# lollcat/fab-torch

Measured on AMD Instinct MI355X. Metric: AIS samples/sec (+ESS), ManyWell-32, 8 intermediate dists, higher is better.
Workload: dtype f32; 1 GPU; headline: ManyWell-32 AIS, RealNVP 10x(16-320-320-32)+InvAffine (seeded default init, last coupling Linears N(0, 0.01^2)), HMC L=5 n_outer=1, M=8 linear beta, alpha=2 (target p^2/q), step-size tuning on; chains_per_gpu=1024, global_chains=1024, parallelism=single GPU

## Files before the change

fab_torch_amd/csrc/flow_r4.h:

```cpp
#pragma once
#include "flow_device.h"
#include "target_device.h"

namespace fab {

constexpr int R4 = 4;
constexpr int R4_DS = MAX_DIM + 4;

struct R4Dims {
    int Kd, Ko, KD;
    int G;
    int o_AW, o_AWT, o_W1, o_W2, o_W3, o_W3T, o_W2T, o_W1T, layer_stride;
};

FAB_HD R4Dims make_r4_dims(const FlowDims& f) {
    R4Dims r;
    r.Kd = pad16(f.d); r.Ko = pad16(2 * f.DOp); r.KD = pad16(f.D);
    r.G = f.Wp / 64;
    int o = 0;
    r.o_AW = o; o += r.KD * 64;
    r.o_AWT = o; o += r.KD * 64;
    r.o_W1 = o; o += r.Kd * f.Wp;
    r.o_W2 = o; o += f.Wp * f.Wp;
    r.o_W3 = o; o += f.Wp * 2 * f.DOp;
    r.o_W3T = o; o += r.Ko * f.Wp;
    r.o_W2T = o; o += f.Wp * f.Wp;
    r.o_W1T = o; o += f.Wp * pad16(f.d);
    r.layer_stride = o;
    return r;
}

struct R4Lds {
    int WS, PN;
    int o_X0, o_X1, o_HA, o_HB, o_PRM, o_DP, o_PART, o_ES, o_V2, o_MASK, total;
    int o_PZ, o_BIAS;
    int o_PF;
};

FAB_HD R4Lds make_r4_lds(const FlowDims& f, bool fused = false) {
    R4Lds l;
    l.WS = fused ? f.Wp + 16 : f.Wp + 4;
    l.PN = f.Wp;
    int o = 0;
    l.o_X0 = o; o += R4 * R4_DS;
    l.o_X1 = o; o += R4 * R4_DS;
    l.o_HA = o; o += R4 * l.WS;
    l.o_HB = o; o += R4 * l.WS;
    l.o_PRM = o; o += R4 * R4_DS;
    l.o_DP = o; o += R4 * R4_DS;
    l.o_PART = o; o += NWAVE * R4 * l.PN;
    l.o_ES = o; o += f.K * R4 * f.DOp;
    l.o_V2 = o; o += f.K * R4 * f.DOp;
    l.o_MASK = o; o += f.K * 2 * NTHREADS;
    l.o_PZ = l.o_BIAS = l.o_PF = 0;
    if (fused) {
        o = (o + 3) & ~3;
        l.o_PZ = o; o += 2 * NWAVE * R4 * 32;
        l.o_BIAS = o; o += (f.K + 1) * r4f_bias_stride(f.Wp);
        o = (o + 3) & ~3;
        l.o_PF = o; o += NWAVE * 64;
    }
    l.total = (o + 3) & ~3;
    return l;
}

__device__ __forceinline__ f32x4 mfma44(float a, float b, f32x4 c) {
    return __builtin_amdgcn_mfma_f32_4x4x1f32(a, b, c, 0, 0, 0);
}

struct Tid4 {
    int tid, wave, lane, arow;
    __device__ __forceinline__ Tid4() {
        tid = threadIdx.x;
        wave = __builtin_amdgcn_readfirstlane(tid >> 6);
        lane = tid & 63;
        arow = lane & 3;
    }
};

template <int NQ, int G>
struct R4Pre {
    float4 b[NQ][G];
};

template <int NQ, int G>
__device__ __forceinline__ void r4_preload(R4Pre<NQ, G>& p, const float4* __restrict__ Bm, int qbase, int nq_valid,
                                           const Tid4& t) {
    const float4* bw = Bm + ((size_t)qbase * G) * 64 + t.lane;
#pragma unroll
    for (int q = 0; q < NQ; ++q)
#pragma unroll
        for (int g = 0; g < G; ++g)
            if (q < nq_valid) p.b[q][g] = bw[(size_t)(q * G + g) * 64];
}

__device__ __forceinline__ void r4_barrier() { asm volatile("s_waitcnt lgkmcnt(0)\n\ts_barrier" ::: "memory"); }

template <int Q0, int Q1, int NQ, int G>
__device__ __forceinline__ void r4_preload_part(R4Pre<NQ, G>& p, const float4* __restrict__ Bm, int qbase, const Tid4& t) {
    const float4* bw = Bm + ((size_t)qbase * G) * 64 + t.lane;
#pragma unroll
    for (int q = Q0; q < Q1 && q < NQ; ++q)
#pragma unroll
        for (int g = 0; g < G; ++g) p.b[q][g] = bw[(size_t)(q * G + g) * 64];
}

struct R4NoNext {
    __device__ __forceinline__ void operator()() const {}
};

template <int G, class BT>
__device__ __forceinline__ void r4_quad(const float4& a, const BT (&b)[G], f32x4 (&acc)[G]) {
#pragma unroll
    for (int g = 0; g < G; ++g) acc[g] = mfma44(a.x, b[g].x, acc[g]);
#pragma unroll
    for (int g = 0; g < G; ++g) acc[g] = mfma44(a.y, b[g].y, acc[g]);
#pragma unroll
    for (int g = 0; g < G; ++g) acc[g] = mfma44(a.z, b[g].z, acc[g]);
#pragma unroll
    for (int g = 0; g < G; ++g) acc[g] = mfma44(a.w, b[g].w, acc[g]);
}

template <int NTWM>
struct R4Ring {
    static constexpr int NQ = 4 * NTWM, RD = NQ < 6 ? NQ : 6;
};

template <int NTWM, int G, class Next>
__device__ __forceinline__ void r4_mma_wide(const float* __restrict__ act, int lda, const float4* __restrict__ Bm,
                                            const R4Pre<R4Ring<NTWM>::RD, G>& pre, const Tid4& t, f32x4 (&acc)[G], Next next) {
    constexpr int NQ = R4Ring<NTWM>::NQ, RD = R4Ring<NTWM>::RD;
    const float* arow = act + t.arow * lda + 16 * NTWM * t.wave;
    const float4* bw = Bm + ((size_t)(4 * NTWM * t.wave) * G) * 64 + t.lane;
    float4 b[RD][G];
#pragma unroll
    for (int q = 0; q < RD; ++q)
#pragma unroll
        for (int g = 0; g < G; ++g) b[q][g] = pre.b[q][g];
    next();
    __builtin_amdgcn_sched_barrier(0);
#pragma unroll
    for (int q = 0; q < NQ; ++q) {
        const float4 a = *reinterpret_cast<const float4*>(arow + 4 * q);
        r4_quad<G>(a, b[q % RD], acc);
        if (q + RD < NQ) {
#pragma unroll
            for (int g = 0; g < G; ++g) b[q % RD][g] = bw[(size_t)((q + RD) * G + g) * 64];
        }
        __builtin_amdgcn_sched_barrier(0);
    }
}

template <int G>
__device__ __forceinline__ void r4_store_part(const f32x4 (&acc)[G], float* __restrict__ part, int PN, const Tid4& t) {
    float* pw = part + (size_t)t.wave * R4 * PN + t.lane;
#pragma unroll
    for (int g = 0; g < G; ++g)
#pragma unroll
        for (int r = 0; r < 4; ++r) pw[r * PN + 64 * g] = acc[g][r];
}

template <int G>
__device__ __forceinline__ void r4_bias_load(float (&bv)[G], const float* __restrict__ bias, const Tid4& t) {
    constexpr int N = 64 * G;
#pragma unroll
    for (int i = 0; i < G; ++i) bv[i] = bias ? bias[(256 * i + t.tid) % N] : 0.f;
}

typedef float f32x2 __attribute__((ext_vector_type(2)));
template <int O0, int O1>
__device__ __forceinline__ f32x2 lds_read2st64(unsigned addr) {
    f32x2 v;
    asm volatile("ds_read2st64_b32 %0, %1 offset0:%2 offset1:%3" : "=v"(v) : "v"(addr), "n"(O0), "n"(O1) : "memory");
    return v;
}
template <int G>
__device__ __forceinline__ void r4_read_partials(const float* part, int PN, int tid, float (&v)[G]) {
    (void)PN;
    const unsigned addr = (unsigned)(size_t)(part + tid);
    f32x2 r[2 * G];
    static_for<0, G>([&](auto ic) {
        constexpr int i = decltype(ic)::value;
        r[2 * i] = lds_read2st64<4 * i, 4 * i + 8 * G>(addr);
        r[2 * i + 1] = lds_read2st64<4 * i + 4 * G, 4 * i + 12 * G>(addr);
    });
    asm volatile("s_waitcnt lgkmcnt(0)" ::: "memory");
#pragma unroll
    for (int k = 0; k < 2 * G; ++k) asm volatile("" : "+v"(r[k]));
#pragma unroll
    for (int i = 0; i < G; ++i) {
        const f32x2 h = r[2 * i] + r[2 * i + 1];
        v[i] = h.x + h.y;
    }
}

struct R4NoPost {
    __device__ __forceinline__ float operator()(int, int, float v) const { return v; }
};

template <int G, int EP, class Post = R4NoPost>
__device__ __forceinline__ void r4_epilogue(const float* __restrict__ part, int PN, const float (&bv)[G],
                                            float* __restrict__ out, int ldo, unsigned* mask, const Tid4& t,
                                            Post post = Post()) {
    constexpr int N = 64 * G;
    unsigned m = EP == 2 ? mask[t.tid] : 0u;
    float v[G];
    if constexpr (G >= 2) {
        r4_read_partials<G>(part, PN, t.tid, v);
#pragma unroll
        for (int i = 0; i < G; ++i) v[i] += bv[i];
    } else {
#pragma unroll
        for (int i = 0; i < G; ++i) {
            const int o = 256 * i + t.tid, row = o / N, col = o - row * N;
            const float* p = part + row * PN + col;
            v[i] = ((p[0] + p[R4 * PN]) + (p[2 * R4 * PN] + p[3 * R4 * PN])) + bv[i];
        }
    }
#pragma unroll
    for (int i = 0; i < G; ++i) {
        const int o = 256 * i + t.tid, row = o / N, col = o - row * N;
        float w = v[i];
        if (EP == 1) { const bool pos = w > 0.f; m |= (pos ? 1u : 0u) << i; w = pos ? w : 0.f; }
        if (EP == 2) w = ((m >> i) & 1u) ? w : 0.f;
        out[row * ldo + col] = post(row, col, w);
    }
    if (EP == 1) mask[t.tid] = m;
}

template <int G>
__device__ __forceinline__ void r4_store_part_rf(const f32x4 (&acc)[G], float* __restrict__ part, const Tid4& t) {
    f32x4* pw = reinterpret_cast<f32x4*>(part + (size_t)t.wave * R4 * 64 * G) + t.lane;
#pragma unroll
    for (int g = 0; g < G; ++g) pw[64 * g] = acc[g];
}
template <int G>
__device__ __forceinline__ void r4_bias_rf(float (&bv)[G], const float* __restrict__ b, const Tid4& t) {
#pragma unroll
    for (int i = 0; i < G; ++i) bv[i] = b[(256 * i + t.tid) >> 2];
}
template <int G, int EP>
__device__ __forceinline__ void r4_epilogue_rf(const float* __restrict__ part, const float (&bv)[G], float* __restrict__ out, int ldo,
                                               unsigned* mask, const Tid4& t) {
    unsigned m = EP == 2 ? mask[t.tid] : 0u;
    float v[G];
    r4_read_partials<G>(part, 64 * G, t.tid, v);
    const int row = t.tid & 3, col0 = t.tid >> 2;
#pragma unroll
    for (int i = 0; i < G; ++i) {
        float w = v[i] + bv[i];
        if (EP == 1) { const bool pos = w > 0.f; m |= (pos ? 1u : 0u) << i; w = pos ? w : 0.f; }
        if (EP == 2) w = ((m >> i) & 1u) ? w : 0.f;
        out[row * ldo + col0 + 64 * i] = w;
    }
    if (EP == 1) mask[t.tid] = m;
}

template <int NTWM, int G, int EP, class Next = R4NoNext>
__device__ __forceinline__ void r4_dense_wide(const float* act, int lda, const float4* Bm,
                                              const R4Pre<R4Ring<NTWM>::RD, G>& pre,
                                              const float (&bv)[G], float* out, int ldo, unsigned* mask, float* part, int PN,
                                              const Tid4& t, Next next = Next()) {
    f32x4 acc[G];
#pragma unroll
    for (int g = 0; g < G; ++g) acc[g] = (f32x4){0.f, 0.f, 0.f, 0.f};
    r4_mma_wide<NTWM, G>(act, lda, Bm, pre, t, acc, next);
    r4_store_part<G>(acc, part, PN, t);
    r4_barrier();
    r4_epilogue<G, EP>(part, PN, bv, out, ldo, mask, t);
    r4_barrier();
}

template <int NTWM, int NT>
struct R4PreT {
    float4 b[NTWM][NT];
};

template <int NTWM, int NT>
__device__ __forceinline__ void r4_preload_n16(R4PreT<NTWM, NT>& p, const float4* __restrict__ Bm, const Tid4& t) {
    const float4* bw = Bm + ((size_t)(NTWM * t.wave) * NT) * 64 + t.lane;
#pragma unroll
    for (int Q = 0; Q < NTWM; ++Q)
#pragma unroll
        for (int ct = 0; ct < NT; ++ct) p.b[Q][ct] = bw[(size_t)(Q * NT + ct) * 64];
}

template <int NTWM, int NT, bool ACC = false, class Next = R4NoNext>
__device__ __forceinline__ void r4_dense_n16(const float* act, int lda, const R4PreT<NTWM, NT>& pre, float* out, int ldo,
                                             float* part, int PN, const Tid4& t, Next next = Next()) {
    constexpr int NSUB = 4 / NT, CW = 16 * NT, NTILE = NTWM * NT;
    static_assert(NT == 1 || NT == 2 || NT == 4, "16, 32 or 64 output columns");
    const int sblk = t.lane / CW, col = t.lane % CW;
    const float* arow = act + t.arow * lda + 16 * NTWM * t.wave + 4 * sblk;
    f32x4 acc0 = (f32x4){0.f, 0.f, 0.f, 0.f}, acc1 = acc0;
#pragma unroll
    for (int T = 0; T < NTILE; ++T) {
        const float4 a = *reinterpret_cast<const float4*>(arow + 4 * NSUB * T);
        const float4 w = pre.b[T / NT][T % NT];
        acc0 = mfma44(a.x, w.x, acc0);
        acc1 = mfma44(a.y, w.y, acc1);
        acc0 = mfma44(a.z, w.z, acc0);
        acc1 = mfma44(a.w, w.w, acc1);
    }
    next();
    acc0 += acc1;
    (void)PN;
    float* pw = part + ((size_t)(t.wave * NSUB + sblk) * R4) * CW + col;
#pragma unroll
    for (int r = 0; r < 4; ++r) pw[r * CW] = acc0[r];
    r4_barrier();
    if (t.tid < R4 * CW) {
        const int row = t.tid / CW, c = t.tid - row * CW;
        const float* p = part + row * CW + c;
        float v[4 * NSUB];
#pragma unroll
        for (int i = 0; i < 4 * NSUB; ++i) v[i] = p[(size_t)i * R4 * CW];
#pragma unroll
        for (int n = 4 * NSUB; n > 1; n >>= 1)
#pragma unroll
            for (int i = 0; i < n / 2; ++i) v[i] = v[2 * i] + v[2 * i + 1];
        if (ACC) out[row * ldo + c] += v[0];
        else out[row * ldo + c] = v[0];
    }
    r4_barrier();
}

template <int NQ, int G, int EP, class Next = R4NoNext, class Post = R4NoPost>
__device__ __forceinline__ void r4_dense_short(const float* act, int lda, int kmax, int nqw, const R4Pre<NQ, G>& pre,
                                               const float (&bv)[G], float* out, int ldo, unsigned* mask, float* part, int PN,
                                               const Tid4& t, Next next = Next(), Post post = Post()) {
    f32x4 acc[G];
#pragma unroll
    for (int g = 0; g < G; ++g) acc[g] = (f32x4){0.f, 0.f, 0.f, 0.f};
    const int q0 = nqw * t.wave;
#pragma unroll
    for (int q = 0; q < NQ; ++q) {
        if (q < nqw) {
            const int k0 = 4 * (q0 + q);
            float4 a = *reinterpret_cast<const float4*>(act + t.arow * lda + k0);
            if (k0 + 0 >= kmax) a.x = 0.f;
            if (k0 + 1 >= kmax) a.y = 0.f;
            if (k0 + 2 >= kmax) a.z = 0.f;
            if (k0 + 3 >= kmax) a.w = 0.f;
            r4_quad<G>(a, pre.b[q], acc);
        }
    }
    next();
    r4_store_part<G>(acc, part, PN, t);
    r4_barrier();
    r4_epilogue<G, EP>(part, PN, bv, out, ldo, mask, t, post);
    r4_barrier();
}

template <int NTWM, int NQS, int NQA, int NT3, int NT1>
__device__ float flow_log_prob_r4(const FlowDims& f, const R4Dims& rd, const R4Lds& l, const float* __restrict__ packed,
                                  float* lds, const Tid4& t, int* grad_off) {
    constexpr int G = NTWM;
    const float* r4base = packed + f.o_r4;
    int cur = l.o_X0, nxt = l.o_X1;
    float* HA = lds + l.o_HA;
    float* HB = lds + l.o_HB;
    float* PRM = lds + l.o_PRM;
    float* DP = lds + l.o_DP;
    float* PART = lds + l.o_PART;
    const bool ew = t.tid < 64;
    const int row = t.tid >> 4, c = t.tid & 15;
    const int nqD = rd.KD / 16, nqd = rd.Kd / 16, nqo = rd.Ko / 16;
    const int qW = 4 * NTWM * t.wave;
    R4Pre<NQA, 1> preA;
    R4PreT<NTWM, NT3> preN3;
    R4PreT<NTWM, NT1> preN1;
    R4Pre<NQS, G> preS;
    constexpr int RD = R4Ring<NTWM>::RD;
    R4Pre<RD, G> preW;
    float bvA[1], bv1[G], bv2[G], bv0[G];
#pragma unroll
    for (int g = 0; g < G; ++g) bv0[g] = 0.f;
    float logq = 0.f;
    {
        const float* Lp = packed + (size_t)(f.K - 1) * f.layer_stride;
        const float* Rp = r4base + (size_t)(f.K - 1) * rd.layer_stride;
        r4_preload<NQA, 1>(preA, reinterpret_cast<const float4*>(Rp + rd.o_AW), nqD * t.wave, nqD, t);
        r4_preload<NQS, G>(preS, reinterpret_cast<const float4*>(Rp + rd.o_W1), nqd * t.wave, nqd, t);
        r4_bias_load<1>(bvA, Lp + f.o_ac, t);
        r4_bias_load<G>(bv1, Lp + f.o_b1, t);
        r4_preload_part<0, 3>(preW, reinterpret_cast<const float4*>(Rp + rd.o_W2), qW, t);
    }
    for (int layer = f.K - 1; layer >= 0; --layer) {
        const float* Lp = packed + (size_t)layer * f.layer_stride;
        const float* Rp = r4base + (size_t)layer * rd.layer_stride;
        unsigned* mk = reinterpret_cast<unsigned*>(lds + l.o_MASK) + (size_t)layer * 2 * NTHREADS;
        const bool tl = layer == f.K - 2;
        if (tl) FAB_TL(f, 0);
        r4_dense_short<NQA, 1, 0>(lds + cur, R4_DS, f.D, nqD, preA, bvA, lds + nxt, R4_DS, nullptr, PART, l.PN, t, [&] {
            r4_preload_part<3, 5>(preW, reinterpret_cast<const float4*>(Rp + rd.o_W2), qW, t);
        });
        logq += Lp[f.o_logS];
        float* Z = lds + nxt;
        if (tl) FAB_TL(f, 1);
        r4_dense_short<NQS, G, 1>(Z, R4_DS, f.d, nqd, preS, bv1, HA, l.WS, mk, PART, l.PN, t, [&] {
            r4_preload_part<5, RD>(preW, reinterpret_cast<const float4*>(Rp + rd.o_W2), qW, t);
        });
        if (tl) FAB_TL(f, 2);
        float b3s[2] = {0.f, 0.f}, b3c[2] = {0.f, 0.f};
        r4_bias_load<G>(bv2, Lp + f.o_b2, t);
        r4_dense_wide<NTWM, G, 1>(HA, l.WS, reinterpret_cast<const float4*>(Rp + rd.o_W2), preW, bv2, HB, l.WS,
                                  mk + NTHREADS, PART, l.PN, t, [&] {
            r4_preload_n16<NTWM, NT3>(preN3, reinterpret_cast<const float4*>(Rp + rd.o_W3), t);
#pragma unroll
            for (int it = 0; it < 2; ++it) {
                const int j = c + 16 * it;
                if (ew && j < f.DO) { b3s[it] = Lp[f.o_b3 + j]; b3c[it] = Lp[f.o_b3 + f.DOp + j]; }
            }
            if (layer > 0) {
                const float* Ln = Lp - f.layer_stride;
                const float* Rn = Rp - rd.layer_stride;
                r4_preload<NQA, 1>(preA, reinterpret_cast<const float4*>(Rn + rd.o_AW), nqD * t.wave, nqD, t);
                r4_preload<NQS, G>(preS, reinterpret_cast<const float4*>(Rn + rd.o_W1), nqd * t.wave, nqd, t);
                r4_bias_load<1>(bvA, Ln + f.o_ac, t);
                r4_bias_load<G>(bv1, Ln + f.o_b1, t);
            } else {
                r4_preload<NQS, G>(preS, reinterpret_cast<const float4*>(Rp + rd.o_W3T), nqo * t.wave, nqo, t);
            }
        });
        if (tl) FAB_TL(f, 3);
        const float4* Wnext = reinterpret_cast<const float4*>(layer > 0 ? Rp - rd.layer_stride + rd.o_W2 : Rp + rd.o_W2T);
        r4_dense_n16<NTWM, NT3>(HB, l.WS, preN3, PRM, R4_DS, PART, l.PN, t, [&] { r4_preload_part<0, 2>(preW, Wnext, qW, t); });
        if (tl) FAB_TL(f, 4);
        r4_preload_part<2, 3>(preW, Wnext, qW, t);
        if (ew) {
            float ssum = 0.f;
#pragma unroll
            for (int it = 0; it < 2; ++it) {
                const int j = c + 16 * it;
                if (j < f.DO) {
                    const float shift = PRM[row * R4_DS + j] + b3s[it];
                    const float s = PRM[row * R4_DS + f.DOp + j] + b3c[it];
                    const float es = expf(-s);
                    const float v2 = (Z[row * R4_DS + f.d + j] - shift) * es;
                    Z[row * R4_DS + f.d + j] = v2;
                    lds[l.o_ES + ((size_t)layer * R4 + row) * f.DOp + j] = es;
                    lds[l.o_V2 + ((size_t)layer * R4 + row) * f.DOp + j] = v2;
                    ssum += s;
                }
            }
            logq += -row16_sum(ssum);
        }
        r4_barrier();
        if (tl) FAB_TL(f, 5);
        const int tmp = cur; cur = nxt; nxt = tmp;
    }
    if (ew) {
        const float* base = packed + f.o_base;
        float* Zc = lds + cur;
        float bsum = 0.f;
        for (int j = c; j < f.D; j += 16) {
            const float ls = base[f.Dp + j];
            const float sc = expf(ls);
            const float zn = (Zc[row * R4_DS + j] - base[j]) / sc;
            bsum += ls + 0.5f * (zn * zn);
            Zc[row * R4_DS + j] = -(zn / sc);
        }
        logq += -0.5f * (float)f.D * 1.8378770664093453f - row16_sum(bsum);
    }
    r4_barrier();
    bvA[0] = 0.f;
    for (int layer = 0; layer < f.K; ++layer) {
        const float* Rp = r4base + (size_t)layer * rd.layer_stride;
        unsigned* mk = reinterpret_cast<unsigned*>(lds + l.o_MASK) + (size_t)layer * 2 * NTHREADS;
        float* Gs = lds + cur;
        const bool tl = layer == 1;
        if (tl) FAB_TL(f, 16);
        r4_preload_part<3, 5>(preW, reinterpret_cast<const float4*>(Rp + rd.o_W2T), qW, t);
        if (layer == 0) {
            if (ew) {
                for (int j = c; j < f.DO; j += 16) {
                    const float g2 = Gs[row * R4_DS + f.d + j];
                    const float es = lds[l.o_ES + (size_t)row * f.DOp + j];
                    const float v2 = lds[l.o_V2 + (size_t)row * f.DOp + j];
                    DP[row * R4_DS + j] = -(g2 * es);
                    DP[row * R4_DS + f.DOp + j] = -(g2 * v2) - 1.f;
                    Gs[row * R4_DS + f.d + j] = g2 * es;
                }
            }
            r4_barrier();
        }
        auto couple = [&](int r, int col, float v) -> float {
            if (layer + 1 < f.K && col >= f.d && col < f.d + f.DO) {
                const int j = col - f.d;
                const float es = lds[l.o_ES + ((size_t)(layer + 1) * R4 + r) * f.DOp + j];
                const float v2 = lds[l.o_V2 + ((size_t)(layer + 1) * R4 + r) * f.DOp + j];
                DP[r * R4_DS + j] = -(v * es);
                DP[r * R4_DS + f.DOp + j] = -(v * v2) - 1.f;
                return v * es;
            }
            return v;
        };
        if (tl) FAB_TL(f, 17);
        r4_dense_short<NQS, G, 2>(DP, R4_DS, 2 * f.DOp, nqo, preS, bv0, HA, l.WS, mk + NTHREADS, PART, l.PN, t, [&] {
            r4_preload_part<5, RD>(preW, reinterpret_cast<const float4*>(Rp + rd.o_W2T), qW, t);
        });
        if (tl) FAB_TL(f, 18);
        r4_dense_wide<NTWM, G, 2>(HA, l.WS, reinterpret_cast<const float4*>(Rp + rd.o_W2T), preW, bv0, HB, l.WS, mk, PART,
                                  l.PN, t, [&] {
            r4_preload_n16<NTWM, NT1>(preN1, reinterpret_cast<const float4*>(Rp + rd.o_W1T), t);
            r4_preload<NQA, 1>(preA, reinterpret_cast<const float4*>(Rp + rd.o_AWT), nqD * t.wave, nqD, t);
            if (layer + 1 < f.K) {
                const float* Rn = Rp + rd.layer_stride;
                r4_preload<NQS, G>(preS, reinterpret_cast<const float4*>(Rn + rd.o_W3T), nqo * t.wave, nqo, t);
            }
        });
        if (tl) FAB_TL(f, 19);
        const float4* Wnext = reinterpret_cast<const float4*>(Rp + rd.layer_stride + rd.o_W2T);
        const bool more = layer + 1 < f.K;
        r4_dense_n16<NTWM, NT1, true>(HB, l.WS, preN1, Gs, R4_DS, PART, l.PN, t, [&] {
            if (more) r4_preload_part<0, 2>(preW, Wnext, qW, t);
        });
        if (tl) FAB_TL(f, 20);
        if (tl) FAB_TL(f, 21);
        r4_dense_short<NQA, 1, 0>(Gs, R4_DS, f.D, nqD, preA, bvA, lds + nxt, R4_DS, nullptr, PART, l.PN, t, [&] {
            if (more) r4_preload_part<2, 3>(preW, Wnext, qW, t);
        }, couple);
        if (tl) FAB_TL(f, 22);
        const int tmp = cur; cur = nxt; nxt = tmp;
    }
    *grad_off = cur;
    return logq;
}


template <int NTWM>
struct R4Stream {
    static constexpr int G = NTWM;
    static constexpr int C = 4 * NTWM + 4;
    static constexpr int RD = C % 6 == 0 ? 6 : (C % 8 == 0 ? 8 : 5);
    static constexpr int IS = 4 * G * 64;
    static constexpr int IA = 0, IW1 = 1, IW2 = 2, IW3 = 2 + 4 * NTWM;
    static constexpr int IW3T = 0, IW2T = 2, IW1T = 2 + 4 * NTWM, IAT = 3 + 4 * NTWM;
    static_assert(C % RD == 0, "ring size must divide the items per layer");
};

template <int NTWM, int EP, int I0, class Ring, class Refill>
__device__ __forceinline__ void r4s_dense_wide(const float* act, int lda, Ring& ring, Refill refill,
                                               const float (&bv)[NTWM], float* out, int ldo, unsigned* mask, float* part,
                                               int PN, const Tid4& t) {
    constexpr int G = NTWM, NQ = 4 * NTWM, RD = R4Stream<NTWM>::RD;
    f32x4 acc[G];
#pragma unroll
    for (int g = 0; g < G; ++g) acc[g] = (f32x4){0.f, 0.f, 0.f, 0.f};
    const float* arow = act + t.arow * lda + 16 * NTWM * t.wave;
    static_for<0, NQ>([&](auto qc) {
        constexpr int q = decltype(qc)::value;
        const float4 a = *reinterpret_cast<const float4*>(arow + 4 * q);
        r4_quad<G>(a, ring[(I0 + q) % RD], acc);
        refill(IC<I0 + q>{});
        __builtin_amdgcn_sched_barrier(0);
    });
    r4_store_part<G>(acc, part, PN, t);
    r4_barrier();
// ... 292 lines not shown
```

fab_torch_amd/csrc/flow_r4f.h:

```cpp
#pragma once
#include "flow_r4.h"
#include "stream_r8.h"

namespace fab {

template <int NTWM, bool FAST = false, int NS_ = 0>
struct R4F {
    static constexpr int G = NTWM;
    static constexpr int NS = NS_;
    static constexpr int NQW = FAST ? 2 * G : 4 * G;
    static constexpr int CR = NQW + 5;
    static constexpr int TL = (NQW + 4) * G + 1;
    static constexpr int I_A = 2, I_W = 3, I_N = NQW + 3;
    static constexpr int SQ0 = 1, SQD = NS > 0 ? (NQW - 5) / NS : 1;
    static constexpr int stash_k(int I) { return (I - I_W - SQ0) / SQD; }
    static constexpr bool is_stash(int I) {
        return NS > 0 && I >= I_W + SQ0 && I < I_N && (I - I_W - SQ0) % SQD == 0 && stash_k(I) < NS;
    }
    static constexpr int stash_item(int k) { return I_W + SQ0 + k * SQD; }
    static constexpr int ntiles(int I) { return I == I_A ? 1 : (I < CR && !is_stash(I) ? G : 0); }
    static constexpr int dma_piece(int I) {
        const int k = I >= I_N ? I - I_N : (I <= I_A ? I + 2 : -1);
        return k >= 0 && k < NS ? k : -1;
    }
    static constexpr bool dma_next_slot(int I) { return I >= I_N; }
    static constexpr int toff(int I) { return I <= I_A ? I * G : (I - 1) * G + 1; }
#ifdef FAB_R4F_RD
    static constexpr int RD = FAB_R4F_RD;
#else
    static constexpr int RD = G >= 5 ? 5 : (G == 4 ? 7 : (FAST ? 9 : 13));
#endif
    static constexpr int C = (CR + RD - 1) / RD * RD;
    static constexpr int E = C - CR;
    static constexpr int STEP = NQW / (E + 1) > 0 ? NQW / (E + 1) : 1;
    static constexpr int vidx(int I) {
        int q = I - I_W;
        q = q < 0 ? 0 : (q > NQW ? NQW : q);
        const int e = q / STEP;
        return I + (e < E ? e : E);
    }
    static constexpr int item_at(int V) {
        for (int I = 0; I < CR; ++I)
            if (vidx(I) == V) return I;
        return -1;
    }
    static constexpr int vtiles(int V) { return item_at(V % C) < 0 ? 0 : ntiles(item_at(V % C)); }
    static constexpr int prev_pos(int I) { return I > 0 ? vidx(I - 1) : vidx(CR - 1) - C; }
    static constexpr int req_hi(int I) { return vidx(I) - 1 + RD; }
    static constexpr int req_lo(int I) { return prev_pos(I) - 1 + RD + 1; }
    static constexpr int inflight_behind(int I) {
        if (NS > 0) return younger(I);
        int n = 0;
        for (int J = vidx(I) + 1; J <= prev_pos(I) - 1 + RD; ++J) n += vtiles(J);
        return n;
    }
    static constexpr int younger(int I) {
        int n = 0;
        for (int step = 1; step <= C; ++step) {
            const int J = ((I - step) % C + C) % C;
            const int pk = dma_piece(J);
            if (pk >= 0) {
                if (is_stash(I) && pk == stash_k(I)) return n;
                n += G;
            }
            const int V = (I - step) - 1 + RD;
            if (!is_stash(I) && V == I) return n;
            n += vtiles(((V % C) + C) % C);
        }
        return 63;
    }
    static_assert(E <= NQW / STEP, "every empty item needs an item of the W x W stage to sit behind");
    static_assert((RD - 1) * G < 64, "vmcnt is a 6-bit counter");
    static_assert(NS == 0 || (E == 0 && !FAST && NS <= 5 && SQD >= 2 && stash_item(NS - 1) + RD - 1 < I_N),
                  "the stash needs a layer without empty items; no stash item within the ring's reach of the short stages");
};


struct R4FAcc {
    f32x4 a[8];
    __device__ __forceinline__ R4FAcc() {
#pragma unroll
        for (int i = 0; i < 8; ++i) a[i] = (f32x4){0.f, 0.f, 0.f, 0.f};
    }
    template <int T, class WT>
    __device__ __forceinline__ void tile(const float4& x, const WT& w) {
        constexpr int o = 4 * (T & 1);
        a[o + 0] = mfma44(x.x, w.x, a[o + 0]);
        a[o + 1] = mfma44(x.y, w.y, a[o + 1]);
        a[o + 2] = mfma44(x.z, w.z, a[o + 2]);
        a[o + 3] = mfma44(x.w, w.w, a[o + 3]);
    }
    __device__ __forceinline__ void store(float* __restrict__ pz, const Tid4& t) const {
        const f32x4 s = ((a[0] + a[1]) + (a[2] + a[3])) + ((a[4] + a[5]) + (a[6] + a[7]));
        float* p = pz + ((size_t)(t.wave * 2 + (t.lane >> 5)) * R4) * 32 + (t.lane & 31);
#pragma unroll
        for (int r = 0; r < 4; ++r) p[r * 32] = s[r];
    }
};

__device__ __forceinline__ float r4f_tree8(const float* __restrict__ pz, int row, int c) {
    const float* p = pz + row * 32 + c;
    float v[8];
#pragma unroll
    for (int i = 0; i < 8; ++i) v[i] = p[(size_t)i * R4 * 32];
    return ((v[0] + v[1]) + (v[2] + v[3])) + ((v[4] + v[5]) + (v[6] + v[7]));
}

__device__ __forceinline__ void r4f_load_bias(const float* __restrict__ src, float* __restrict__ dst, int nfloats, int tid) {
    const float4* s4 = reinterpret_cast<const float4*>(src);
    float4* d4 = reinterpret_cast<float4*>(dst);
    for (int e = tid; e < nfloats / 4; e += NTHREADS) d4[e] = s4[e];
}

template <int NTWM, bool FAST = false, int NS = 0>
struct R4FRing {
    using S = R4F<NTWM, FAST, NS>;
    static constexpr int G = S::G, RD = S::RD, C = S::C;
    f32x4 r[RD][G];
    const float4 *spG, *sp1;
    unsigned voff0, voff1;
    unsigned stash_m0;
    const float4* stash_rd;
    __device__ __forceinline__ R4FRing(const float4* base, const Tid4& t, float* stash = nullptr)
        : spG(base + (size_t)t.wave * G * 64), sp1(base + (size_t)t.wave * 64), voff0((unsigned)t.lane * 16u),
          voff1((unsigned)t.lane * 16u + 4096u),
          stash_m0((unsigned)__builtin_amdgcn_readfirstlane((int)(unsigned)(size_t)stash + t.wave * (NS * G * 1024))),
          stash_rd(reinterpret_cast<const float4*>(stash) + (size_t)t.wave * (NS * G * 64) + t.lane) {
        if constexpr (NS == 0) static_for<0, RD - 1>([&](auto vc) { request<decltype(vc)::value>(); });
        else {
            static_for<0, RD - 1>([&](auto pc) {
                constexpr int P = decltype(pc)::value - (RD - 1);
                request<P - 1 + RD>();
                constexpr int I = P + C;
                if constexpr (S::dma_piece(I) >= 0) request_dma<S::dma_piece(I), false>();
            });
        }
    }
    template <int K, bool NEXT>
    __device__ __forceinline__ void request_dma() {
        constexpr int I = S::stash_item(K);
        const float4* b0 = spG + ((size_t)(NEXT ? 1 : 0) * S::TL + S::toff(I)) * 4 * 64;
        const unsigned long long bu = (unsigned long long)b0;
        const float4* b = reinterpret_cast<const float4*>(
            ((unsigned long long)(unsigned)__builtin_amdgcn_readfirstlane((int)(bu >> 32)) << 32) |
            (unsigned long long)(unsigned)__builtin_amdgcn_readfirstlane((int)(bu & 0xffffffffull)));
        const unsigned dst = stash_m0 + K * G * 1024;
        static_assert(G >= 2 && G <= 5, "");
        if constexpr (G == 2)
            asm volatile("s_mov_b32 m0, %2\n\ts_nop 4\n\tglobal_load_lds_dwordx4 %0, %1 offset:0\n\t"
                         "global_load_lds_dwordx4 %0, %1 offset:1024" :: "v"(voff0), "s"(b), "s"(dst) : "memory", "m0");
        else if constexpr (G == 3)
            asm volatile("s_mov_b32 m0, %2\n\ts_nop 4\n\tglobal_load_lds_dwordx4 %0, %1 offset:0\n\t"
                         "global_load_lds_dwordx4 %0, %1 offset:1024\n\tglobal_load_lds_dwordx4 %0, %1 offset:2048"
                         :: "v"(voff0), "s"(b), "s"(dst) : "memory", "m0");
        else
            asm volatile("s_mov_b32 m0, %2\n\ts_nop 4\n\tglobal_load_lds_dwordx4 %0, %1 offset:0\n\t"
                         "global_load_lds_dwordx4 %0, %1 offset:1024\n\tglobal_load_lds_dwordx4 %0, %1 offset:2048\n\t"
                         "global_load_lds_dwordx4 %0, %1 offset:3072" :: "v"(voff0), "s"(b), "s"(dst) : "memory", "m0");
        if constexpr (G == 5)
            asm volatile("s_mov_b32 m0, %2\n\ts_nop 0\n\tglobal_load_lds_dwordx4 %0, %1 offset:0"
                         :: "v"(voff1), "s"(b), "s"(dst + 4096u) : "memory", "m0");
    }
    template <int I>
    __device__ __forceinline__ void wait_stash(IC<I>) {
        constexpr int N = S::inflight_behind(I);
        static_assert(S::is_stash(I) && N >= 0 && N < 64, "vmcnt is a 6-bit counter");
        asm volatile("s_waitcnt vmcnt(%0)" :: "n"(N) : "memory");
    }
    template <int I>
    __device__ __forceinline__ void read_stash(IC<I>, float4 (&w)[G]) const {
        constexpr int K = S::stash_k(I);
#pragma unroll
        for (int g = 0; g < G; ++g) w[g] = stash_rd[(K * G + g) * 64];
    }
    template <int V>
    __device__ __forceinline__ void request() {
        constexpr int I = S::item_at(V % C);
        if constexpr (I >= 0) {
            constexpr int n = S::ntiles(I), SL = V % RD;
            const float4* b0 = (n == G ? spG : sp1) + ((size_t)(V / C) * S::TL + S::toff(I)) * 4 * 64;
            const unsigned long long bu = (unsigned long long)b0;
            const float4* b = reinterpret_cast<const float4*>(
                ((unsigned long long)(unsigned)__builtin_amdgcn_readfirstlane((int)(bu >> 32)) << 32) |
                (unsigned long long)(unsigned)__builtin_amdgcn_readfirstlane((int)(bu & 0xffffffffull)));
            static_for<0, n>([&](auto gc) {
                constexpr int g = decltype(gc)::value;
                if constexpr (g == 0) s8_load_first<0>(r[SL][0], voff0, b);
                else if constexpr (g < 4) s8_load<g * 1024>(r[SL][g], voff0, b);
                else s8_load<(g - 4) * 1024>(r[SL][g], voff1, b);
            });
        }
    }
    template <int I>
    static constexpr int slot(IC<I>) { return S::vidx(I) % RD; }
    template <int I>
    __device__ __forceinline__ void wait(IC<I>) {
        constexpr int SL = S::vidx(I) % RD, N = S::inflight_behind(I);
        static_assert(!S::is_stash(I) && N >= 0 && N < 64, "vmcnt is a 6-bit counter");
        if constexpr (S::ntiles(I) == 1) asm volatile("s_waitcnt vmcnt(%1)" : "+a"(r[SL][0]) : "n"(N));
        else if constexpr (G == 2) asm volatile("s_waitcnt vmcnt(%2)" : "+a"(r[SL][0]), "+a"(r[SL][1]) : "n"(N));
        else if constexpr (G == 4)
            asm volatile("s_waitcnt vmcnt(%4)" : "+a"(r[SL][0]), "+a"(r[SL][1]), "+a"(r[SL][2]), "+a"(r[SL][3]) : "n"(N));
        else
            asm volatile("s_waitcnt vmcnt(%5)"
                         : "+a"(r[SL][0]), "+a"(r[SL][1]), "+a"(r[SL][2]), "+a"(r[SL][3]), "+a"(r[SL][4])
                         : "n"(N));
        __builtin_amdgcn_sched_barrier(0);
    }
    template <int I>
    __device__ __forceinline__ void refill(IC<I>) {
        __builtin_amdgcn_sched_barrier(0);
        static_for<S::req_lo(I), S::req_hi(I) + 1>([&](auto pc) { request<decltype(pc)::value>(); });
        if constexpr (S::dma_piece(I) >= 0) request_dma<S::dma_piece(I), S::dma_next_slot(I)>();
        __builtin_amdgcn_sched_barrier(0);
    }
    __device__ __forceinline__ void next_layer() { spG += (size_t)S::TL * 4 * 64; sp1 += (size_t)S::TL * 4 * 64; }
    __device__ __forceinline__ void drain() {
        static_for<0, RD>([&](auto sc) {
            constexpr int SL = decltype(sc)::value;
            static_for<0, G>([&](auto gc) { asm volatile("s_waitcnt vmcnt(0)" : "+a"(r[SL][decltype(gc)::value])); });
        });
    }
};

template <int NTWM, int I0, class Ring>
__device__ __forceinline__ void r4f_short_mma(const float4& a0, const float4& a1, Ring& ring, float* part, int PN, const Tid4& t) {
    constexpr int G = NTWM, RD = Ring::RD;
    f32x4 acc0[G], acc1[G];
#pragma unroll
    for (int g = 0; g < G; ++g) { acc0[g] = (f32x4){0.f, 0.f, 0.f, 0.f}; acc1[g] = acc0[g]; }
    ring.wait(IC<I0>{});
    r4_quad<G>(a0, ring.r[ring.slot(IC<I0>{})], acc0);
    ring.refill(IC<I0>{});
    __builtin_amdgcn_sched_barrier(0);
    ring.wait(IC<I0 + 1>{});
    r4_quad<G>(a1, ring.r[ring.slot(IC<I0 + 1>{})], acc1);
    ring.refill(IC<I0 + 1>{});
    __builtin_amdgcn_sched_barrier(0);
#pragma unroll
    for (int g = 0; g < G; ++g) acc0[g] += acc1[g];
    (void)PN;
    r4_store_part_rf<G>(acc0, part, t);
}

template <int NTWM, int EP, class Ring>
__device__ __forceinline__ void r4f_dense_wide(const float* act, int lda, Ring& ring, const float* __restrict__ bias, float* out,
                                               int ldo, unsigned* mask, float* part, int PN, const Tid4& t) {
    using S = typename Ring::S;
    constexpr int G = NTWM, NQ = 4 * NTWM, I0 = S::I_W;
    f32x4 acc[G];
#pragma unroll
    for (int g = 0; g < G; ++g) acc[g] = (f32x4){0.f, 0.f, 0.f, 0.f};
    const float* arow = act + t.arow * lda + 16 * NTWM * t.wave;
    float4 ws[2][G];
    static_for<0, NQ>([&](auto qc) {
        constexpr int q = decltype(qc)::value;
        const float4 a = *reinterpret_cast<const float4*>(arow + 4 * q);
        if constexpr (S::is_stash(I0 + q)) {
            r4_quad<G>(a, ws[S::stash_k(I0 + q) & 1], acc);
        } else {
            ring.wait(IC<I0 + q>{});
            r4_quad<G>(a, ring.r[ring.slot(IC<I0 + q>{})], acc);
        }
        ring.refill(IC<I0 + q>{});
        if constexpr (q + 1 < NQ && S::is_stash(I0 + q + 1)) {
            ring.wait_stash(IC<I0 + q + 1>{});
            ring.read_stash(IC<I0 + q + 1>{}, ws[S::stash_k(I0 + q + 1) & 1]);
        }
        __builtin_amdgcn_sched_barrier(0);
    });
    (void)PN;
    r4_store_part_rf<G>(acc, part, t);
    float bv[G];
    if (bias) r4_bias_rf<G>(bv, bias, t);
    else {
#pragma unroll
        for (int g = 0; g < G; ++g) bv[g] = 0.f;
    }
    r4_barrier();
    r4_epilogue_rf<G, EP>(part, bv, out, ldo, mask, t);
    r4_barrier();
}

typedef short s16x4 __attribute__((ext_vector_type(4)));
typedef float f32x2v __attribute__((ext_vector_type(2)));
__device__ __forceinline__ s16x4 r4f_bf16x4(const float4& a) {
    union { unsigned u[2]; s16x4 v; } c;
    c.u[0] = cvt_pk_bf16(a.x, a.y);
    c.u[1] = cvt_pk_bf16(a.z, a.w);
    return c.v;
}
template <int NTWM, int EP, class Ring>
__device__ __forceinline__ void r4f_dense_wide_bf16(const float* act, int lda, Ring& ring, const float* __restrict__ bias, float* out,
                                                    int ldo, unsigned* mask, float* part, const Tid4& t) {
    using S = typename Ring::S;
    constexpr int G = NTWM, NI = 2 * NTWM, I0 = S::I_W;
    f32x4 acc0[G], acc1[G];
#pragma unroll
    for (int g = 0; g < G; ++g) { acc0[g] = (f32x4){0.f, 0.f, 0.f, 0.f}; acc1[g] = acc0[g]; }
    const float* arow = act + t.arow * lda + 16 * NTWM * t.wave;
    static_for<0, NI>([&](auto ic) {
        constexpr int i = decltype(ic)::value;
        const s16x4 a0 = r4f_bf16x4(*reinterpret_cast<const float4*>(arow + 8 * i));
        const s16x4 a1 = r4f_bf16x4(*reinterpret_cast<const float4*>(arow + 8 * i + 4));
        ring.wait(IC<I0 + i>{});
        constexpr int SL = Ring::slot(IC<I0 + i>{});
#pragma unroll
        for (int g = 0; g < G; ++g) {
            const f32x4 w = ring.r[SL][g];
            acc0[g] = __builtin_amdgcn_mfma_f32_4x4x4bf16_1k(a0, __builtin_bit_cast(s16x4, (f32x2v)__builtin_shufflevector(w, w, 0, 1)),
                                                             acc0[g], 0, 0, 0);
        }
#pragma unroll
        for (int g = 0; g < G; ++g) {
            const f32x4 w = ring.r[SL][g];
            acc1[g] = __builtin_amdgcn_mfma_f32_4x4x4bf16_1k(a1, __builtin_bit_cast(s16x4, (f32x2v)__builtin_shufflevector(w, w, 2, 3)),
                                                             acc1[g], 0, 0, 0);
        }
#pragma unroll
        for (int g = 0; g < G; ++g) asm volatile("" : : "a"(ring.r[SL][g]));
#pragma unroll
        for (int g = 0; g < G; ++g) asm volatile("" : "+v"(acc0[g]), "+v"(acc1[g]) : "v"(a0), "v"(a1));
        ring.refill(IC<I0 + i>{});
        __builtin_amdgcn_sched_barrier(0);
    });
#pragma unroll
    for (int g = 0; g < G; ++g) acc0[g] += acc1[g];
    r4_store_part_rf<G>(acc0, part, t);
    float bv[G];
    if (bias) r4_bias_rf<G>(bv, bias, t);
    else {
#pragma unroll
        for (int g = 0; g < G; ++g) bv[g] = 0.f;
    }
    r4_barrier();
    r4_epilogue_rf<G, EP>(part, bv, out, ldo, mask, t);
    r4_barrier();
}

template <int NTWM, class Ring>
__device__ __forceinline__ void r4f_narrow_mma(const float* act, int lda, Ring& ring, R4FAcc& p, const Tid4& t) {
    using S = typename Ring::S;
    constexpr int G = NTWM, RD = S::RD, I0 = S::I_N;
    const float* arow = act + t.arow * lda + 16 * NTWM * t.wave + 4 * (t.lane >> 5);
    static_for<0, 2 * G>([&](auto tc) {
        constexpr int T = decltype(tc)::value;
        const float4 a = *reinterpret_cast<const float4*>(arow + 8 * T);
        if constexpr (T % G == 0) ring.wait(IC<I0 + T / G>{});
        p.template tile<T>(a, ring.r[ring.slot(IC<I0 + T / G>{})][T % G]);
        if constexpr (T % G == G - 1) {
            ring.refill(IC<I0 + T / G>{});
            __builtin_amdgcn_sched_barrier(0);
        }
    });
}

#ifndef FAB_R4F_PF_AHEAD
#define FAB_R4F_PF_AHEAD 2
#endif
template <int TL>
__device__ __forceinline__ unsigned r4f_prefetch_line(const Tid4& t) {
    constexpr unsigned NL = (unsigned)TL * 32u;
    unsigned nsh = (gridDim.x + 7u) >> 3;
    nsh = nsh > 32u ? 32u : nsh;
    if (nsh * 64u * (unsigned)t.wave >= NL) return ~0u;
    unsigned line = (blockIdx.x >> 3) % nsh + nsh * (unsigned)(64 * t.wave + t.lane);
    line = line < NL ? line : NL - 1u;
    return line * 128u;
}
template <int TL>
__device__ __forceinline__ void r4f_prefetch_l2(const float* junk, unsigned voff, const char* img, int slot, int nslots) {
    if constexpr (FAB_R4F_PF_AHEAD > 0) {
        if (voff == ~0u) return;
        int ts = slot + FAB_R4F_PF_AHEAD;
        ts = ts >= nslots ? ts - nslots : ts;
        const unsigned long long bu = (unsigned long long)(img + (size_t)ts * ((size_t)TL * 4096));
        const char* b = reinterpret_cast<const char*>(
            ((unsigned long long)(unsigned)__builtin_amdgcn_readfirstlane((int)(bu >> 32)) << 32) |
            (unsigned long long)(unsigned)__builtin_amdgcn_readfirstlane((int)(bu & 0xffffffffull)));
        const unsigned m0v = (unsigned)__builtin_amdgcn_readfirstlane((int)(unsigned)(size_t)junk);
        asm volatile("s_mov_b32 m0, %2\n\ts_nop 4\n\tglobal_load_lds_dword %0, %1" :: "v"(voff), "s"(b), "s"(m0v) : "memory", "m0");
    }
}

template <int NTWM, bool FAST = false, int NS = 0>
__device__ float flow_log_prob_r4f(const FlowDims& f, const R4Lds& l, const float* __restrict__ packed, float* lds,
                                   const Tid4& t, int* grad_off, float* stash = nullptr) {
    using S = R4F<NTWM, FAST, NS>;
    constexpr int G = NTWM, RD = S::RD;
    float* X = lds + l.o_X0;
    float* HA = lds + l.o_HA;
    float* HB = lds + l.o_HB;
    float* DP = lds + l.o_DP;
    float* PART = lds + l.o_PART;
    float* PZ = lds + l.o_PZ;
    const float* BT = lds + l.o_BIAS;
    const int BS = r4f_bias_stride(f.Wp);
    const bool ew = t.tid < 64;
    const int row = t.tid >> 4, c = t.tid & 15;
    const int zrow = t.tid >> 5, zc = t.tid & 31;
    const int sblk = t.lane >> 5;
    R4FRing<NTWM, FAST, NS> ring(reinterpret_cast<const float4*>(packed + (FAST ? f.o_r4fh : f.o_r4f)), t, stash);
    const char* pf_img = reinterpret_cast<const char*>(packed + (FAST ? f.o_r4fh : f.o_r4f));
    const float* pf_junk = lds + l.o_PF + 64 * t.wave;
    const unsigned pf_voff = r4f_prefetch_line<S::TL>(t);
    int pf_slot = 0;
    float logq = 0.f;
#pragma unroll 1
    for (int layer = f.K - 1; layer >= 0; --layer) {
        const float* bt = BT + (size_t)layer * BS;
        unsigned* mk = reinterpret_cast<unsigned*>(lds + l.o_MASK) + (size_t)layer * 2 * NTHREADS;
        const bool tl = layer == f.K - 2;
        if (tl) FAB_TL(f, 0);
        {
            const float* xr = X + t.arow * R4_DS + 8 * t.wave;
            const float4 a0 = *reinterpret_cast<const float4*>(xr), a1 = *reinterpret_cast<const float4*>(xr + 4);
#ifdef FAB_R4F_WAVETL
            long long wt[8];
#define FAB_WT(k) do { __builtin_amdgcn_sched_barrier(0); wt[k] = (long long)__builtin_amdgcn_s_memtime(); __builtin_amdgcn_sched_barrier(0); } while (0)
            FAB_WT(0);
            {
                f32x4 acc0[G], acc1[G];
#pragma unroll
                for (int g = 0; g < G; ++g) { acc0[g] = (f32x4){0.f, 0.f, 0.f, 0.f}; acc1[g] = acc0[g]; }
                ring.wait(IC<0>{});
                FAB_WT(1);
                r4_quad<G>(a0, ring.r[ring.slot(IC<0>{})], acc0);
                FAB_WT(2);
                ring.refill(IC<0>{});
                FAB_WT(3);
                ring.wait(IC<1>{});
                r4_quad<G>(a1, ring.r[ring.slot(IC<1>{})], acc1);
                FAB_WT(4);
                ring.refill(IC<1>{});
                FAB_WT(5);
#pragma unroll
                for (int g = 0; g < G; ++g) acc0[g] += acc1[g];
                r4_store_part_rf<G>(acc0, PART, t);
            }
#else
            r4f_short_mma<NTWM, 0>(a0, a1, ring, PART, l.PN, t);
#endif
            R4FAcc z;
            ring.wait(IC<S::I_A>{});
            z.template tile<0>(sblk ? a1 : a0, ring.r[ring.slot(IC<S::I_A>{})][0]);
            ring.refill(IC<S::I_A>{});
            r4f_prefetch_l2<S::TL>(pf_junk, pf_voff, pf_img, pf_slot++, 2 * f.K);
#ifdef FAB_R4F_WAVETL
            FAB_WT(6);
#endif
            z.store(PZ, t);
            float bv[G];
            r4_bias_rf<G>(bv, bt, t);
            r4_barrier();
#ifdef FAB_R4F_WAVETL
            FAB_WT(7);
            if (tl && f.timeline && blockIdx.x == 0 && t.lane == 0) {
#pragma unroll
                for (int k = 0; k < 8; ++k) f.timeline[32 + 8 * t.wave + k] = wt[k];
            }
#endif
            float zv = 0.f;
            if (t.tid < 128) zv = r4f_tree8(PZ, zrow, zc) + bt[2 * f.Wp + zc];
            r4_epilogue_rf<G, 1>(PART, bv, HA, l.WS, mk, t);
            if (t.tid < 128) X[zrow * R4_DS + zc] = zv;
            r4_barrier();
        }
        logq += bt[2 * f.Wp + 64];
        if (tl) FAB_TL(f, 1);
        if constexpr (FAST) r4f_dense_wide_bf16<NTWM, 1>(HA, l.WS, ring, bt + f.Wp, HB, l.WS, mk + NTHREADS, PART, t);
        else r4f_dense_wide<NTWM, 1>(HA, l.WS, ring, bt + f.Wp, HB, l.WS, mk + NTHREADS, PART, l.PN, t);
        if (tl) FAB_TL(f, 3);
        {
            R4FAcc p;
            r4f_narrow_mma<NTWM>(HB, l.WS, ring, p, t);
            p.store(PZ, t);
            r4_barrier();
            if (ew) {
                float ssum = 0.f;
                if (c < f.DO) {
                    const float shift = r4f_tree8(PZ, row, c) + bt[2 * f.Wp + 32 + c];
                    const float s = r4f_tree8(PZ, row, 16 + c) + bt[2 * f.Wp + 48 + c];
                    const float es = expf(-s);
                    const float v2 = (X[row * R4_DS + f.d + c] - shift) * es;
                    X[row * R4_DS + f.d + c] = v2;
                    lds[l.o_ES + ((size_t)layer * R4 + row) * f.DOp + c] = es;
                    lds[l.o_V2 + ((size_t)layer * R4 + row) * f.DOp + c] = v2;
                    ssum = s;
                }
                logq += -row16_sum(ssum);
            }
            r4_barrier();
        }
        if (tl) FAB_TL(f, 5);
        ring.next_layer();
    }
    if (ew) {
        const float* base = packed + f.o_base;
        float bsum = 0.f;
        for (int j = c; j < f.D; j += 16) {
            const float ls = base[f.Dp + j];
            const float sc = expf(ls);
            const float zn = (X[row * R4_DS + j] - base[j]) / sc;
            bsum += ls + 0.5f * (zn * zn);
            float g = -(zn / sc);
            if (j >= f.d) {
                const int jj = j - f.d;
                const float es = lds[l.o_ES + (size_t)row * f.DOp + jj];
                const float v2 = lds[l.o_V2 + (size_t)row * f.DOp + jj];
                DP[row * R4_DS + jj] = -(g * es);
                DP[row * R4_DS + f.DOp + jj] = -(g * v2) - 1.f;
                g = g * es;
            }
            X[row * R4_DS + j] = g;
        }
        logq += -0.5f * (float)f.D * 1.8378770664093453f - row16_sum(bsum);
    }
    r4_barrier();
#pragma unroll 1
    for (int layer = 0; layer < f.K; ++layer) {
        unsigned* mk = reinterpret_cast<unsigned*>(lds + l.o_MASK) + (size_t)layer * 2 * NTHREADS;
        const bool tl = layer == 1;
        if (tl) FAB_TL(f, 16);
        f32x4 atile;
        {
            const float* dr = DP + t.arow * R4_DS + 8 * t.wave;
            const float4 a0 = *reinterpret_cast<const float4*>(dr), a1 = *reinterpret_cast<const float4*>(dr + 4);
            r4f_short_mma<NTWM, 0>(a0, a1, ring, PART, l.PN, t);
            ring.wait(IC<S::I_A>{});
            {
                const f32x4 tsrc = ring.r[ring.slot(IC<S::I_A>{})][0];
                float ax = tsrc.x, ay = tsrc.y, az = tsrc.z, aw = tsrc.w;
                asm volatile("" : "+v"(ax), "+v"(ay), "+v"(az), "+v"(aw));
                atile = (f32x4){ax, ay, az, aw};
            }
            ring.refill(IC<S::I_A>{});
            r4f_prefetch_l2<S::TL>(pf_junk, pf_voff, pf_img, pf_slot++, 2 * f.K);
            float bv[G];
#pragma unroll
            for (int g = 0; g < G; ++g) bv[g] = 0.f;
            r4_barrier();
            r4_epilogue_rf<G, 2>(PART, bv, HA, l.WS, mk + NTHREADS, t);
            r4_barrier();
        }
        if (tl) FAB_TL(f, 18);
        if constexpr (FAST) r4f_dense_wide_bf16<NTWM, 2>(HA, l.WS, ring, nullptr, HB, l.WS, mk, PART, t);
        else r4f_dense_wide<NTWM, 2>(HA, l.WS, ring, nullptr, HB, l.WS, mk, PART, l.PN, t);
        if (tl) FAB_TL(f, 19);
        {
            R4FAcc p;
            r4f_narrow_mma<NTWM>(HB, l.WS, ring, p, t);
            const float4 ag = *reinterpret_cast<const float4*>(X + t.arow * R4_DS + 8 * t.wave + 4 * sblk);
            p.template tile<0>(ag, atile);
            p.store(PZ, t);
            r4_barrier();
            if (t.tid < 128) {
                float v = r4f_tree8(PZ, zrow, zc);
                if (layer + 1 < f.K && zc >= f.d && zc < f.d + f.DO) {
                    const int j = zc - f.d;
                    const float es = lds[l.o_ES + ((size_t)(layer + 1) * R4 + zrow) * f.DOp + j];
                    const float v2 = lds[l.o_V2 + ((size_t)(layer + 1) * R4 + zrow) * f.DOp + j];
                    DP[zrow * R4_DS + j] = -(v * es);
                    DP[zrow * R4_DS + f.DOp + j] = -(v * v2) - 1.f;
                    v = v * es;
                }
                X[zrow * R4_DS + zc] = v;
            }
            r4_barrier();
        }
        if (tl) FAB_TL(f, 22);
        ring.next_layer();
    }
    ring.drain();
    *grad_off = l.o_X0;
    return logq;
}

template <int NTWM>
__device__ float flow_sample_r4f(const FlowDims& f, const R4Lds& l, const float* __restrict__ packed, float* lds, const Tid4& t,
                                 int* x_off) {
    using S = R4F<NTWM>;
    constexpr int G = NTWM, RD = S::RD;
    float* X = lds + l.o_X0;
    float* HA = lds + l.o_HA;
    float* HB = lds + l.o_HB;
    float* PART = lds + l.o_PART;
    float* PZ = lds + l.o_PZ;
    const float* BT = lds + l.o_BIAS;
    const int BS = r4f_bias_stride(f.Wp);
    const bool ew = t.tid < 64;
    const int row = t.tid >> 4, c = t.tid & 15;
    const int zrow = t.tid >> 5, zc = t.tid & 31;
    const int sblk = t.lane >> 5;
    unsigned* mk = reinterpret_cast<unsigned*>(lds + l.o_MASK);
    R4FRing<NTWM> ring(reinterpret_cast<const float4*>(packed + f.o_r4f) + (size_t)(2 * f.K + 1) * S::TL * 4 * 64, t);
    float logq = 0.f;
    if (ew) {
        const float* base = packed + f.o_base;
        float bsum = 0.f;
        for (int j = c; j < f.D; j += 16) {
            const float e = X[row * R4_DS + j];
            const float ls = base[f.Dp + j];
            X[row * R4_DS + j] = base[j] + expf(ls) * e;
            bsum += ls + 0.5f * (e * e);
        }
        logq = -0.5f * (float)f.D * 1.8378770664093453f - row16_sum(bsum);
    }
    r4_barrier();
    auto s1 = [&](const float* bt) {
        const float* xr = X + t.arow * R4_DS + 8 * t.wave;
        const float4 a0 = *reinterpret_cast<const float4*>(xr), a1 = *reinterpret_cast<const float4*>(xr + 4);
        r4f_short_mma<NTWM, 0>(a0, a1, ring, PART, l.PN, t);
        R4FAcc z;
        ring.wait(IC<S::I_A>{});
        z.template tile<0>(sblk ? a1 : a0, ring.r[ring.slot(IC<S::I_A>{})][0]);
        ring.refill(IC<S::I_A>{});
        z.store(PZ, t);
        float bv[G];
        r4_bias_rf<G>(bv, bt, t);
        r4_barrier();
        float zv = 0.f;
        if (t.tid < 128) zv = r4f_tree8(PZ, zrow, zc) + bt[2 * f.Wp + zc];
        r4_epilogue_rf<G, 1>(PART, bv, HA, l.WS, mk, t);
        if (t.tid < 128) X[zrow * R4_DS + zc] = zv;
        r4_barrier();
        logq -= -bt[2 * f.Wp + 64];
    };
#pragma unroll 1
    for (int v = 0; v < f.K; ++v) {
        const float* bt = BT + (size_t)v * BS;
        s1(bt);
        r4f_dense_wide<NTWM, 1>(HA, l.WS, ring, bt + f.Wp, HB, l.WS, mk + NTHREADS, PART, l.PN, t);
        {
            R4FAcc p;
            r4f_narrow_mma<NTWM>(HB, l.WS, ring, p, t);
            p.store(PZ, t);
            r4_barrier();
            if (ew) {
                float ssum = 0.f;
                if (c < f.DO) {
                    const float shift = r4f_tree8(PZ, row, c) + bt[2 * f.Wp + 32 + c];
                    const float s = r4f_tree8(PZ, row, 16 + c) + bt[2 * f.Wp + 48 + c];
                    X[row * R4_DS + f.d + c] = X[row * R4_DS + f.d + c] * expf(s) + shift;
                    ssum = s;
                }
                logq -= row16_sum(ssum);
            }
            r4_barrier();
        }
        ring.next_layer();
    }
    s1(BT + (size_t)f.K * BS);
    ring.drain();
    *x_off = l.o_X0;
    return logq;
}

int option(int key);
bool r4f_lds_fits(const FlowDims& f);
static inline bool use_r4_fused(const FlowDims& f) {
    if (f.o_r4f < 0 || f.NTW / 4 < 2 || f.NTW / 4 > 5 || option(FABHIP_OPT_R4_STREAM) < 2) return false;
    return r4f_lds_fits(f);
}

}
```

Before: 245,600 AIS samples/s.

## Replace post-epilogue barriers with wave-local handover via wave-owned output columns

Changes the epilogue so each wave reduces and writes only its own contiguous column block of the hidden activation, which is also the slice it will read next. That lets the block-wide barrier after each epilogue become a per-wave LDS wait. A second partials buffer (PART2) is added so consecutive dense layers do not race on the same scratch space once the barrier is gone, and partial reads use paired stride-64 LDS loads. This costs extra LDS and relies on the assumption that the next matmul only reads wave-local activations. Any cross-wave read, such as the X writes by threads below 128, now depends on later barriers, which is a correctness risk.

```diff
diff --git a/fab_torch_amd/csrc/flow_r4.h b/fab_torch_amd/csrc/flow_r4.h
--- a/fab_torch_amd/csrc/flow_r4.h
+++ b/fab_torch_amd/csrc/flow_r4.h
@@ -35,6 +35,7 @@
     int o_X0, o_X1, o_HA, o_HB, o_PRM, o_DP, o_PART, o_ES, o_V2, o_MASK, total;
     int o_PZ, o_BIAS;
     int o_PF;
+    int o_PART2;
 };
 
 FAB_HD R4Lds make_r4_lds(const FlowDims& f, bool fused = false) {
@@ -53,8 +54,10 @@
     l.o_V2 = o; o += f.K * R4 * f.DOp;
     l.o_MASK = o; o += f.K * 2 * NTHREADS;
     l.o_PZ = l.o_BIAS = l.o_PF = 0;
+    l.o_PART2 = l.o_PART;
     if (fused) {
         o = (o + 3) & ~3;
+        l.o_PART2 = o; o += NWAVE * R4 * l.PN;
         l.o_PZ = o; o += 2 * NWAVE * R4 * 32;
         l.o_BIAS = o; o += (f.K + 1) * r4f_bias_stride(f.Wp);
         o = (o + 3) & ~3;
@@ -237,24 +240,44 @@
 template <int G>
 __device__ __forceinline__ void r4_bias_rf(float (&bv)[G], const float* __restrict__ b, const Tid4& t) {
 #pragma unroll
-    for (int i = 0; i < G; ++i) bv[i] = b[(256 * i + t.tid) >> 2];
+    for (int i = 0; i < G; ++i) bv[i] = b[16 * G * t.wave + (t.lane >> 2) + 16 * i];
+}
+template <int G>
+__device__ __forceinline__ void r4_read_partials_rf(const float* part, const Tid4& t, float (&v)[G]) {
+    const unsigned addr = (unsigned)(size_t)(part + 64 * G * t.wave + t.lane);
+    f32x2 r[2 * G];
+    static_for<0, G>([&](auto ic) {
+        constexpr int i = decltype(ic)::value;
+        r[2 * i] = lds_read2st64<i, i + 8 * G>(addr);
+        r[2 * i + 1] = lds_read2st64<i + 4 * G, i + 12 * G>(addr);
+    });
+    asm volatile("s_waitcnt lgkmcnt(0)" ::: "memory");
+#pragma unroll
+    for (int k = 0; k < 2 * G; ++k) asm volatile("" : "+v"(r[k]));
+#pragma unroll
+    for (int i = 0; i < G; ++i) {
+        const f32x2 h = r[2 * i] + r[2 * i + 1];
+        v[i] = h.x + h.y;
+    }
 }
 template <int G, int EP>
 __device__ __forceinline__ void r4_epilogue_rf(const float* __restrict__ part, const float (&bv)[G], float* __restrict__ out, int ldo,
                                                unsigned* mask, const Tid4& t) {
+    static_assert(13 * G <= 256, "ds_read2st64_b32 offsets (i + 12 G at most) are 8 bits");
     unsigned m = EP == 2 ? mask[t.tid] : 0u;
     float v[G];
-    r4_read_partials<G>(part, 64 * G, t.tid, v);
-    const int row = t.tid & 3, col0 = t.tid >> 2;
+    r4_read_partials_rf<G>(part, t, v);
+    const int row = t.lane & 3, col0 = 16 * G * t.wave + (t.lane >> 2);
 #pragma unroll
     for (int i = 0; i < G; ++i) {
         float w = v[i] + bv[i];
         if (EP == 1) { const bool pos = w > 0.f; m |= (pos ? 1u : 0u) << i; w = pos ? w : 0.f; }
         if (EP == 2) w = ((m >> i) & 1u) ? w : 0.f;
-        out[row * ldo + col0 + 64 * i] = w;
+        out[row * ldo + col0 + 16 * i] = w;
     }
     if (EP == 1) mask[t.tid] = m;
 }
+__device__ __forceinline__ void r4_wave_handover() { asm volatile("s_waitcnt lgkmcnt(0)" ::: "memory"); }
 
 template <int NTWM, int G, int EP, class Next = R4NoNext>
 __device__ __forceinline__ void r4_dense_wide(const float* act, int lda, const float4* Bm,
diff --git a/fab_torch_amd/csrc/flow_r4f.h b/fab_torch_amd/csrc/flow_r4f.h
--- a/fab_torch_amd/csrc/flow_r4f.h
+++ b/fab_torch_amd/csrc/flow_r4f.h
@@ -279,7 +279,7 @@
     }
     r4_barrier();
     r4_epilogue_rf<G, EP>(part, bv, out, ldo, mask, t);
-    r4_barrier();
+    r4_wave_handover();
 }
 
 typedef short s16x4 __attribute__((ext_vector_type(4)));
@@ -335,7 +335,7 @@
     }
     r4_barrier();
     r4_epilogue_rf<G, EP>(part, bv, out, ldo, mask, t);
-    r4_barrier();
+    r4_wave_handover();
 }
 
 template <int NTWM, class Ring>
@@ -393,6 +393,7 @@
     float* HB = lds + l.o_HB;
     float* DP = lds + l.o_DP;
     float* PART = lds + l.o_PART;
+    float* PART2 = lds + l.o_PART2;
     float* PZ = lds + l.o_PZ;
     const float* BT = lds + l.o_BIAS;
     const int BS = r4f_bias_stride(f.Wp);
@@ -464,12 +465,12 @@
             if (t.tid < 128) zv = r4f_tree8(PZ, zrow, zc) + bt[2 * f.Wp + zc];
             r4_epilogue_rf<G, 1>(PART, bv, HA, l.WS, mk, t);
             if (t.tid < 128) X[zrow * R4_DS + zc] = zv;
-            r4_barrier();
+            r4_wave_handover();
         }
         logq += bt[2 * f.Wp + 64];
         if (tl) FAB_TL(f, 1);
-        if constexpr (FAST) r4f_dense_wide_bf16<NTWM, 1>(HA, l.WS, ring, bt + f.Wp, HB, l.WS, mk + NTHREADS, PART, t);
-        else r4f_dense_wide<NTWM, 1>(HA, l.WS, ring, bt + f.Wp, HB, l.WS, mk + NTHREADS, PART, l.PN, t);
+        if constexpr (FAST) r4f_dense_wide_bf16<NTWM, 1>(HA, l.WS, ring, bt + f.Wp, HB, l.WS, mk + NTHREADS, PART2, t);
+        else r4f_dense_wide<NTWM, 1>(HA, l.WS, ring, bt + f.Wp, HB, l.WS, mk + NTHREADS, PART2, l.PN, t);
         if (tl) FAB_TL(f, 3);
         {
             R4FAcc p;
@@ -541,11 +542,11 @@
             for (int g = 0; g < G; ++g) bv[g] = 0.f;
             r4_barrier();
             r4_epilogue_rf<G, 2>(PART, bv, HA, l.WS, mk + NTHREADS, t);
-            r4_barrier();
+            r4_wave_handover();
         }
         if (tl) FAB_TL(f, 18);
-        if constexpr (FAST) r4f_dense_wide_bf16<NTWM, 2>(HA, l.WS, ring, nullptr, HB, l.WS, mk, PART, t);
-        else r4f_dense_wide<NTWM, 2>(HA, l.WS, ring, nullptr, HB, l.WS, mk, PART, l.PN, t);
+        if constexpr (FAST) r4f_dense_wide_bf16<NTWM, 2>(HA, l.WS, ring, nullptr, HB, l.WS, mk, PART2, t);
+        else r4f_dense_wide<NTWM, 2>(HA, l.WS, ring, nullptr, HB, l.WS, mk, PART2, l.PN, t);
         if (tl) FAB_TL(f, 19);
         {
             R4FAcc p;
@@ -585,6 +586,7 @@
     float* HA = lds + l.o_HA;
     float* HB = lds + l.o_HB;
     float* PART = lds + l.o_PART;
+    float* PART2 = lds + l.o_PART2;
     float* PZ = lds + l.o_PZ;
     const float* BT = lds + l.o_BIAS;
     const int BS = r4f_bias_stride(f.Wp);
@@ -623,14 +625,14 @@
         if (t.tid < 128) zv = r4f_tree8(PZ, zrow, zc) + bt[2 * f.Wp + zc];
         r4_epilogue_rf<G, 1>(PART, bv, HA, l.WS, mk, t);
         if (t.tid < 128) X[zrow * R4_DS + zc] = zv;
-        r4_barrier();
+        r4_wave_handover();
         logq -= -bt[2 * f.Wp + 64];
     };
 #pragma unroll 1
     for (int v = 0; v < f.K; ++v) {
         const float* bt = BT + (size_t)v * BS;
         s1(bt);
-        r4f_dense_wide<NTWM, 1>(HA, l.WS, ring, bt + f.Wp, HB, l.WS, mk + NTHREADS, PART, l.PN, t);
+        r4f_dense_wide<NTWM, 1>(HA, l.WS, ring, bt + f.Wp, HB, l.WS, mk + NTHREADS, PART2, l.PN, t);
         {
             R4FAcc p;
             r4f_narrow_mma<NTWM>(HB, l.WS, ring, p, t);
@@ -651,6 +653,7 @@
         ring.next_layer();
     }
     s1(BT + (size_t)f.K * BS);
+    r4_barrier();
     ring.drain();
     *x_off = l.o_X0;
     return logq;
```

Result: faster. 252,100 AIS samples/s, median of 6 (+2.6%).
